# emreatilgan/P-Companion

Measured on AMD Instinct MI355X. Metric: triplets/sec (Product2Vec pretrain step: gather+fwd+bwd+Adam) + P-Companion joint step under `joint`, higher is better.
Workload: dtype f32

## Files before the change

### include/pcompanion_hip.h

```cpp
#ifndef PCOMPANION_HIP_H
#define PCOMPANION_HIP_H

#include <stddef.h>
#include <stdint.h>

#ifdef __cplusplus
extern "C" {
#endif

#define PC_OK 0
#define PC_EINVAL (-1)
#define PC_ESHAPE (-2)
#define PC_EWORKSPACE (-3)
#define PC_EBATCHNORM (-4)
#define PC_ECOMM (-5)

#define PC_D 128
#define PC_H 256
#define PC_HEADS 4
#define PC_L 64
#define PC_MAX_SEG 4
#define PC_BN_SYNC_DOUBLES (PC_MAX_SEG * 2 * 256 + PC_MAX_SEG)

#define PC_ABI_VERSION 8
int pc_abi_version(void);
enum { PC_OPT_SIDE_QUEUE = 1, PC_OPT_SORTED_TABLE_GRADIENTS = 2, PC_OPT_BN_FINALIZE_SIDE = 3, PC_OPT_FUSED_LOSS = 4,
       PC_OPT_FUSED_OUT_CHAIN = 5, PC_OPT_BN_FINALIZE_RIDES = 6, PC_OPT_DW0_STAGED_H = 7 };
int pc_set_option(int option, int value);
int pc_get_option(int option, int* value);
int pc_release_device_state(void);
enum {
    PC_FLAG_EXP_NO_MFMA = 1, PC_FLAG_EXP_NO_SPLIT = 2, PC_FLAG_EXP_NO_LDSREAD = 4, PC_FLAG_EXP_NO_DMA = 8,
    PC_FLAG_EXP_NO_SLAB = 16, PC_FLAG_EXP_STAGGER = 32, PC_FLAG_EXP_DMA_L2 = 64, PC_FLAG_NT_TIMING = 128,
    PC_FLAG_JOINT_TIMING = 256, PC_FLAG_CHAIN_TIMING = 512, PC_FLAG_EXP_NO_BARRIER = 1024, PC_FLAG_EXP_NO_VMWAIT = 2048
};
unsigned pc_build_flags(void);

typedef struct {
    float p;
    uint64_t seed, offset;
} pc_dropout;

typedef struct {
    float *w0, *b0, *gamma, *beta, *w3, *b3, *w5, *b5;
    float *in_proj_w, *in_proj_b, *out_proj_w, *out_proj_b;
    float *running_mean, *running_var;
    int64_t *num_batches_tracked;
    pc_dropout dropout;
    int dim;
} pc_p2v_tensors;

typedef struct {
    int nseg;
    int start[PC_MAX_SEG + 1];
    int count[PC_MAX_SEG];
    int weighted_row;
    float weight;
    const float *row_weight;
    int row_weight_start, row_weight_rows;
} pc_segments;

typedef struct {
    float *h0;
    float *a2;
    float *bn_mean;
    float *bn_invstd;
    float *bn_scale;
    float *bn_shift;
    float *a1;
} pc_ffn_saved;

size_t pc_p2v_ffn_workspace_bytes(int rows);
int pc_p2v_ffn_forward_train(const pc_p2v_tensors *p, const float *table, const int32_t *idx,
                             int rows, const pc_segments *seg, int update_running,
                             float *y, const pc_ffn_saved *saved, void *ws, size_t ws_bytes,
                             void *stream);

int pc_p2v_ffn_forward_eval(const pc_p2v_tensors *p, const float *table, const int32_t *idx,
                            int rows, float *y, void *ws, size_t ws_bytes, void *stream);

// ... 596 lines not shown
```

### p_companion_amd/_lib.py

```python
import ctypes
import os

_HERE = os.path.dirname(os.path.abspath(__file__))
LIB_PATH = os.path.join(_HERE, "libpcompanion_hip.so")
if os.environ.get("PC_DEV_LIB"):
    import sys as _sys
    LIB_PATH = os.path.abspath(os.environ["PC_DEV_LIB"])
    print(f"[p_companion_amd] PC_DEV_LIB: loading {LIB_PATH} instead of the in-tree library (developer A/B run)", file=_sys.stderr, flush=True)

c_f32p = ctypes.c_void_p
c_i32p = ctypes.c_void_p
PC_MAX_SEG = 4
D, H, HEADS, L = 128, 256, 4, 64

_ERR = {-1: "PC_EINVAL (null pointer / bad size)", -2: "PC_ESHAPE (unsupported dimension/alignment)",
        -3: "PC_EWORKSPACE (workspace too small)",
        -4: "PC_EBATCHNORM (a BatchNorm call group of one row in training mode)",
        -5: "PC_ECOMM (RCCL could not be loaded, or a communicator call failed)"}


class HipKernelError(RuntimeError):
    pass


# ... 1 lines not shown
    _fields_ = [("p", ctypes.c_float), ("seed", ctypes.c_uint64), ("offset", ctypes.c_uint64)]


class P2VTensors(ctypes.Structure):
    _fields_ = [(n, ctypes.c_void_p) for n in (
        "w0", "b0", "gamma", "beta", "w3", "b3", "w5", "b5", "in_proj_w", "in_proj_b", "out_proj_w",
        "out_proj_b", "running_mean", "running_var", "num_batches_tracked")] + [("dropout", Dropout), ("dim", ctypes.c_int)]


class Segments(ctypes.Structure):
    _fields_ = [("nseg", ctypes.c_int), ("start", ctypes.c_int * (PC_MAX_SEG + 1)),
                ("count", ctypes.c_int * PC_MAX_SEG), ("weighted_row", ctypes.c_int), ("weight", ctypes.c_float),
                ("row_weight", ctypes.c_void_p), ("row_weight_start", ctypes.c_int), ("row_weight_rows", ctypes.c_int)]


class FfnSaved(ctypes.Structure):
    _fields_ = [(n, ctypes.c_void_p) for n in ("h0", "a2", "bn_mean", "bn_invstd", "bn_scale", "bn_shift", "a1")]


class AttnSaved(ctypes.Structure):
    _fields_ = [(n, ctypes.c_void_p) for n in ("q", "qt", "probs", "c", "sp", "ctx")]


class JointTensors(ctypes.Structure):
    _fields_ = [(n, ctypes.c_void_p) for n in (
        "product_table", "enc_w", "enc_b", "dec_w", "dec_b", "typ_w", "typ_b", "itm_w", "itm_b",
        "query_types", "comp_types")] + [("dropout", Dropout)]


class JointSaved(ctypes.Structure):
    _fields_ = [(n, ctypes.c_void_p) for n in ("h", "c", "pi", "tp")]


_vp, _i, _sz, _f, _d, _u64, _i64 = (ctypes.c_void_p, ctypes.c_int, ctypes.c_size_t, ctypes.c_float,
                                    ctypes.c_double, ctypes.c_uint64, ctypes.c_int64)
_P = ctypes.POINTER

class AdamFused(ctypes.Structure):
    _fields_ = [("param", ctypes.c_void_p), ("grad", ctypes.c_void_p), ("exp_avg", ctypes.c_void_p), ("exp_avg_sq", ctypes.c_void_p),
                ("n", ctypes.c_size_t), ("step_count", ctypes.c_void_p), ("t", ctypes.c_int64),
                ("lr", ctypes.c_double), ("beta1", ctypes.c_double), ("beta2", ctypes.c_double), ("eps", ctypes.c_double)]


class RowWhere(ctypes.Structure):
    _fields_ = [(n, ctypes.c_void_p) for n in ("value", "lo", "hi", "flags", "need", "deny")]


PC_OPT_SIDE_QUEUE = 1
PC_OPT_FUSED_OUT_CHAIN = 5
PC_OPT_FUSED_LOSS = 4
PC_OPT_BN_FINALIZE_SIDE = 3
PC_OPT_BN_FINALIZE_RIDES = 6
PC_OPT_DW0_STAGED_H = 7
PC_OPT_SORTED_TABLE_GRADIENTS = 2

SIGNATURES = {
    "pc_abi_version": (_i, []),
    "pc_build_flags": (ctypes.c_uint, []),
    "pc_set_option": (_i, [_i, _i]),
    "pc_get_option": (_i, [_i, ctypes.POINTER(ctypes.c_int)]),
    "pc_release_device_state": (_i, []),
    "pc_p2v_ffn_workspace_bytes": (_sz, [_i]),
    "pc_p2v_ffn_forward_train": (_i, [_P(P2VTensors), _vp, _vp, _i, _P(Segments), _i, _vp, _P(FfnSaved), _vp, _sz, _vp]),
    "pc_p2v_ffn_forward_eval": (_i, [_P(P2VTensors), _vp, _vp, _i, _vp, _vp, _sz, _vp]),
    "pc_p2v_ffn_backward": (_i, [_P(P2VTensors), _P(P2VTensors), _vp, _vp, _i, _P(Segments), _vp, _P(FfnSaved),
                                 _vp, _i, _vp, _sz, _vp]),
    "pc_p2v_attention_workspace_bytes": (_sz, [_i, _i]),
    "pc_p2v_attention_workspace_bytes_dim": (_sz, [_i, _i, _i]),
    "pc_p2v_attention_forward": (_i, [_P(P2VTensors), _vp, _vp, _i, _i, _vp, _P(AttnSaved), _vp, _sz, _vp]),
    "pc_p2v_attention_backward": (_i, [_P(P2VTensors), _P(P2VTensors), _vp, _vp, _i, _i, _vp, _P(AttnSaved), _vp,
                                       _vp, _i, _vp, _sz, _vp]),
    "pc_p2v_attention_forward_masked": (_i, [_P(P2VTensors), _vp, _vp, _vp, _i, _i, _vp, _P(AttnSaved), _vp, _sz, _vp]),
    "pc_p2v_attention_backward_masked": (_i, [_P(P2VTensors), _P(P2VTensors), _vp, _vp, _vp, _i, _i, _vp, _P(AttnSaved), _vp,
                                              _vp, _i, _vp, _sz, _vp]),
    "pc_p2v_train_step_compact_masked": (_i, [_P(P2VTensors), _P(P2VTensors), _vp, _vp, _vp, _vp, _vp, _i, _vp, _i, _i, _i, _f,
                                              _vp, _vp, _vp, _vp, _vp, _vp, _sz, _vp]),
    "pc_p2v_train_step_unique_masked": (_i, [_P(P2VTensors), _P(P2VTensors), _vp, _vp, _vp, _vp, _vp, _vp, _vp, _i, _i, _vp, _vp,
                                             _vp, _i, _i, _i, _f, _vp, _vp, _vp, _vp, _vp, _vp, _sz, _P(AdamFused), _vp]),
    "pc_p2v_export_workspace_bytes": (_sz, [_i, _i]),
    "pc_p2v_export_embeddings": (_i, [_P(P2VTensors), _vp, _i64, _vp, _vp, _vp, _vp, _i, _vp, _sz, _vp]),
    "pc_p2v_triplet_loss": (_i, [_vp, _vp, _vp, _i, _i, _f, _vp, _vp, _vp, _vp, _vp, _vp, _vp]),
    "pc_p2v_triplet_loss_dim": (_i, [_vp, _vp, _vp, _i, _i, _i, _f, _vp, _vp, _vp, _vp, _vp, _vp, _vp]),
    "pc_adam_step": (_i, [_vp, _vp, _vp, _vp, _sz, _vp, _vp, _d, _d, _d, _d, _vp]),
    "pc_adam_step_at": (_i, [_vp, _vp, _vp, _vp, _sz, _vp, _i64, _d, _d, _d, _d, _vp]),
    "pc_p2v_train_step_workspace_bytes": (_sz, [_i, _i, _i]),
    "pc_p2v_train_step_workspace_bytes_dim": (_sz, [_i, _i, _i, _i]),
    "pc_p2v_train_step": (_i, [_P(P2VTensors), _P(P2VTensors), _vp, _vp, _vp, _vp, _vp, _i, _i, _i, _f, _vp, _vp,
                               _vp, _vp, _vp, _vp, _sz, _vp]),
    "pc_p2v_train_step_compact": (_i, [_P(P2VTensors), _P(P2VTensors), _vp, _vp, _vp, _vp, _vp, _i, _vp, _i, _i, _i, _f,
                                       _vp, _vp, _vp, _vp, _vp, _vp, _sz, _vp]),
    "pc_p2v_train_step_unique_adam": (_i, [_P(P2VTensors), _P(P2VTensors), _vp, _vp, _vp, _vp, _vp, _vp, _i, _vp, _vp, _vp, _i, _i,
                                           _i, _f, _vp, _vp, _vp, _vp, _vp, _vp, _sz, _P(AdamFused), _vp]),
    "pc_p2v_concat_step_rows": (_i, [_vp, _vp, _vp, _vp, _vp, _i, _i, _i, _vp, _i, _vp]),
    "pc_p2v_train_step_unique_rows": (_i, [_P(P2VTensors), _P(P2VTensors), _vp, _vp, _vp, _vp, _i, _vp, _vp, _vp, _i, _i,
                                           _i, _f, _vp, _vp, _vp, _vp, _vp, _vp, _sz, _P(AdamFused), _vp]),
    "pc_p2v_train_step_unique": (_i, [_P(P2VTensors), _P(P2VTensors), _vp, _vp, _vp, _vp, _vp, _vp, _i, _vp, _vp, _vp, _i, _i,
                                      _i, _f, _vp, _vp, _vp, _vp, _vp, _i, _vp, _vp, _vp, _vp, _sz, _vp]),
    "pc_build_similarity_batch_unique_scratch_bytes": (_sz, [_i, _i]),
    "pc_build_similarity_batch_unique": (_i, [_vp, _i, _vp, _vp, _vp, _vp, _vp, _i, _i, _i, _u64, _u64, _i, _vp, _vp, _vp,
                                              _vp, _vp, _vp, _vp, _vp, _vp, _vp, _sz, _vp]),
    "pc_p2v_train_step_compact_sync": (_i, [_P(P2VTensors), _P(P2VTensors), _vp, _vp, _vp, _vp, _vp, _i, _vp, _i, _i, _i,
                                            _f, _vp, _vp, _vp, _vp, _i, _vp, _vp, _vp, _vp, _sz, _vp]),
    "pc_build_similarity_batch_compact": (_i, [_vp, _i, _vp, _vp, _vp, _vp, _vp, _i, _i, _i, _u64, _u64, _vp, _vp, _vp,
                                               _vp, _vp, _vp, _vp]),
    "pc_profile_create": (_i, [_i, _P(ctypes.c_void_p)]),
    "pc_profile_destroy": (_i, [_vp]),
# ... 210 lines not shown
```

### p_companion_amd/csrc/common.h

```cpp
#pragma once
#include <hip/hip_runtime.h>
#include <stdint.h>
#include "../../include/pcompanion_hip.h"

typedef float f32x16 __attribute__((ext_vector_type(16)));
typedef float f32x4 __attribute__((ext_vector_type(4)));

#define PC_WAVE 64

#define PC_HIP_TRY(expr)                          \
    do {                                          \
        hipError_t _e = (expr);                   \
        if (_e != hipSuccess) return (int)_e;     \
    } while (0)

#define PC_TRY(expr)                 \
    do {                             \
        int _r = (expr);             \
        if (_r != 0) return _r;      \
    } while (0)

extern thread_local int pc_tls_launch_err;
#define PC_LAUNCH(...)                                                           \
    do {                                                                         \
// ... 466 lines not shown
};
struct TnReduceGroup {
    const float* slabs[PC_TN_RGROUP]; float* dW[PC_TN_RGROUP]; float* db[PC_TN_RGROUP];
    int nsplit[PC_TN_RGROUP], n_w[PC_TN_RGROUP], n_b[PC_TN_RGROUP], accumulate[PC_TN_RGROUP], block0[PC_TN_RGROUP + 1], n;
    AdamRider ad;
};
#define PC_FORK_EVENTS 3
struct PcFork { hipStream_t side; hipEvent_t fork[PC_FORK_EVENTS]; hipEvent_t join[PC_FORK_EVENTS]; int pending; };
PcFork* pc_fork_get(hipStream_t main_st);
int pc_fork_begin(PcFork* f, int i, hipStream_t main_st);
int pc_fork_mark(PcFork* f, int i);
int pc_fork_wait(PcFork* f, int i, hipStream_t main_st);
int pc_fork_join(PcFork* f, int i, hipStream_t main_st);
struct TnDefer { TnReduceGroup r; int rblocks; PcFork* fork; int bn_finalized; const pc_adam_fused* adam; };
static_assert(sizeof(TnGroup) <= 4096, "kernel argument segment");
int launch_gemm_tn_group(const TnArgs* args, int n, const TnReduceJob* extra, int n_extra, hipStream_t st,
                         TnDefer* defer = nullptr);
int launch_tn_reduce_deferred(TnDefer* d, hipStream_t st);
static inline void tn_defer_init(TnDefer* d) { d->r = TnReduceGroup{}; d->rblocks = 0; d->fork = nullptr; d->bn_finalized = 0; d->adam = nullptr; }
int scatter_add_slab_blocks(int table_rows, int rows, int width);
int launch_scatter_add_slabs(const int32_t* idx, int rows, int width, int table_rows, const float* src, float* slabs,
                             hipStream_t st);

struct WsCarver {
    char* base; size_t total;
    explicit WsCarver(void* b) : base(static_cast<char*>(b)), total(0) {}
    void* bytes(size_t n) {
        void* p = base ? base + total : nullptr;
        total += (n + 255) & ~(size_t)255;
        return p;
    }
    float* floats(size_t n) { return static_cast<float*>(bytes(n * sizeof(float))); }
};

static inline void joint_fields(const pc_joint_tensors* t, float* (&out)[10]) {
    float* const f[10] = {t->itm_w, t->itm_b, t->typ_w, t->typ_b, t->dec_w, t->dec_b, t->enc_w, t->enc_b, t->comp_types, t->query_types};
    for (int i = 0; i < 10; i++) out[i] = f[i];
}
static inline bool joint_tensors_ok(const pc_joint_tensors* t, bool need_table) {
    if (!t || (need_table && !t->product_table)) return false;
    float* f[10];
    joint_fields(t, f);
    for (float* x : f)
        if (!x) return false;
    return true;
}

int pc_opt_sorted_tables();
int pc_opt_bn_finalize_side();
int pc_opt_bn_finalize_rides();
int pc_opt_fused_loss();
int pc_opt_fused_out_chain();
int pc_opt_dw0_staged_h();
int triplet_loss_launch(const float* a, const float* p, const float* n, int batch, int k_neg, int dim, float margin,
                        float* loss, float* d_pos, float* d_neg, float* da, float* dp, float* dn, void* stream, int with_mean);
int launch_dropout(const float* x, size_t n, const pc_dropout& d, unsigned stream_id, float* y, hipStream_t st);
int launch_transpose(const float* in, int rows, int cols, float* out, hipStream_t st);
struct FfnCall {
    const pc_p2v_tensors *p = nullptr, *g = nullptr;
    const float* table = nullptr;
    const int32_t* idx = nullptr;
    int rows = 0;
    const pc_segments* seg = nullptr;
    const pc_ffn_saved* sv = nullptr;
    void* ws = nullptr; size_t ws_bytes = 0; void* stream = nullptr;
    double* local_sums = nullptr; const double* global_sums = nullptr;
    int update_running = 0; float* y = nullptr;
    const TransposeBatch* ride = nullptr;
    const float* dy = nullptr; float* dx = nullptr;
    int with_dx = 0, transposed = 0;
    int accumulate = 0;
    TnDefer* defer = nullptr;
};
int ffn_forward_part1(const FfnCall& c);
int ffn_forward_part2(const FfnCall& c);
int ffn_backward_part1(const FfnCall& c);
int ffn_backward_part2(const FfnCall& c);
int ffn_transposes(const pc_p2v_tensors* p, void* ws, int rows, int with_dx, TransposeBatch* tb);
int attention_transposes(const pc_p2v_tensors* p, void* ws, int B, int N, int key_rows, TransposeBatch* tb, float* zero_bk);
struct AttnCall {
    const pc_p2v_tensors* p = nullptr;
    const float *query = nullptr, *keys = nullptr;
    int B = 0, N = 0, key_rows = 0;
    const int32_t* slot_row = nullptr;
    const pc_attn_saved* sv = nullptr;
    void* ws = nullptr; size_t ws_bytes = 0; void* stream = nullptr;
    bool transposed = false;
    bool masked = false;
    const uint8_t* key_pad = nullptr;
    float* out = nullptr;
    const pc_p2v_tensors* g = nullptr;
    int pad_row = -1;
    const float* dout = nullptr;
    float *dquery = nullptr, *dkeys = nullptr;
    int accumulate = 0;
    const int32_t *ref_off = nullptr, *ref_slot = nullptr;
    TnDefer* defer = nullptr;
    const HingeMeanJob* rider = nullptr;
    const LossPro* loss = nullptr;
    const NtArgs* fwd_out_chain = nullptr;
    NtArgs* defer_out_chain = nullptr;
};
int attention_forward_impl(const AttnCall& c);
int attention_backward_impl(const AttnCall& c);

static inline NtArgs nt_plain(const float* A, int lda, const float* W, int ldw, const float* bias, float* C, int ldc, int M,
// ... 9 lines not shown
```

### p_companion_amd/csrc/gemm_tn.hip

```cpp
#include <atomic>
#include <mutex>
#include <type_traits>
#include "common.h"
#include "bn_finalize.h"
#include "lds_dma.h"

#define TM 128
#define TK 32

__device__ __forceinline__ float4 bn_bwd_z4(float4 z, const float4& h, float zm, const float4& mu, const float4& is,
                                            const float4& sc, const float4& c1, const float4& c2) {
    z.x = sc.x * (z.x - zm * (c1.x + (h.x - mu.x) * is.x * c2.x));
    z.y = sc.y * (z.y - zm * (c1.y + (h.y - mu.y) * is.y * c2.y));
    z.z = sc.z * (z.z - zm * (c1.z + (h.z - mu.z) * is.z * c2.z));
    z.w = sc.w * (z.w - zm * (c1.w + (h.w - mu.w) * is.w * c2.w));
    return z;
}

__device__ __forceinline__ void tn_small_body(const TnArgs& a, int tiles_i, int nsplit, int rows_per_split, int bid) {
    __shared__ __attribute__((aligned(16))) float smem[2][2][TK * TM];

    const int tid = threadIdx.x, lane = tid & 63, w = tid >> 6, wo = w >> 1, wi = w & 1;
    const int split = bid % nsplit;
    const int tile = bid / nsplit;
// ... 89 lines not shown
            const float x0 = As[k * TM], x1 = As[k * TM + 32];
            if (vz0 && vx0) acc[0][0] = mfma32(z0, x0, acc[0][0]);
            if (vz0 && vx1) acc[0][1] = mfma32(z0, x1, acc[0][1]);
            if (vz1 && vx0) acc[1][0] = mfma32(z1, x0, acc[1][0]);
            if (vz1 && vx1) acc[1][1] = mfma32(z1, x1, acc[1][1]);
        }
        if (c + 1 < nchunk) lstore(cur ^ 1);
        __syncthreads();
    }

    float* slab = a.slabs + (size_t)split * ((size_t)a.No * a.Ni + a.No);
#pragma unroll
    for (int mt = 0; mt < 2; mt++)
#pragma unroll
        for (int nt = 0; nt < 2; nt++) {
            const int i = i0 + wi * 64 + nt * 32 + (lane & 31);
#pragma unroll
            for (int reg = 0; reg < 16; reg++) {
                const int o = o0 + wo * 64 + mt * 32 + (reg & 3) + 8 * (reg >> 2) + 4 * (lane >> 5);
                if (o < a.No && i < a.Ni) slab[(size_t)o * a.Ni + i] = acc[mt][nt][reg];
            }
        }
    if (a.db && i0 == 0) {
        float* red = &smem[0][0][0];
        *reinterpret_cast<float4*>(&red[lrow * TM + lcol]) = dbacc;
        __syncthreads();
        if (tid < TM && o0 + tid < a.No) {
            float s = 0.f;
#pragma unroll
            for (int g = 0; g < 8; g++) s += red[g * TM + tid];
            slab[(size_t)a.No * a.Ni + o0 + tid] = s;
        }
    }
}

__global__ __launch_bounds__(256, 2) void gemm_tn_kernel(TnArgs a, int tiles_i, int nsplit, int rows_per_split) {
    tn_small_body(a, tiles_i, nsplit, rows_per_split, blockIdx.x);
}

__global__ __launch_bounds__(256, 2) void gemm_tn_group_kernel(TnGroup g) {
    const int b = blockIdx.x;
    int j = 0;
#pragma unroll
    for (int i = 1; i < PC_TN_GROUP; i++) j += (i < g.n && b >= g.block0[i]) ? 1 : 0;
    tn_small_body(g.a[j], g.tiles_i[j], g.nsplit[j], g.rps[j], b - g.block0[j]);
}

__device__ __attribute__((aligned(64))) float pc_tn_zero_chunk[16];

struct TnNoRider {};
typedef float tn_v4f __attribute__((ext_vector_type(4)));
__device__ __forceinline__ void tn_tie_h(tn_v4f (&h)[4]) { asm volatile("" : "+v"(h[0]), "+v"(h[1]), "+v"(h[2]), "+v"(h[3])::"memory"); }
__device__ __forceinline__ void tn_tie_h(tn_v4f (&h)[2]) { asm volatile("" : "+v"(h[0]), "+v"(h[1])::"memory"); }
#ifdef PC_EXP_DW0_REGH_16X3
#define PC_TN_REGH_ALL 1
#else
#define PC_TN_REGH_ALL 0
#endif
template <int WO, int WI, int TO, int TI, int TKC, int NST, bool APRO, bool ZPRO, bool RIDER = false>
__global__ __launch_bounds__(64 * WO * WI, WO * WI / 4) void gemm_tn8_kernel(TnArgs a, int nsplit, int rows_per_split, int halves,
                                                                             size_t slab_half_off,
                                                                             std::conditional_t<RIDER, TnRider, TnNoRider> rider) {
    constexpr bool REGH = ZPRO && (TKC == 32 || (PC_TN_REGH_ALL && WO == 4));
    static_assert(!REGH || (!APRO && !RIDER), "register H is a form of the ZPRO loader");
    constexpr int NWV = WO * WI, THREADS = 64 * NWV;
    constexpr int NO = WO * TO * 32, NI = WI * TI * 32;
    constexpr int ZRS = NO == 256 ? 260 : NO, ARS = NI == 256 ? 260 : NI;
    constexpr bool ZSW = NO == 128, ASW = NI == 128;
    static_assert((NO == 128 || NO == 256) && (NI == 128 || NI == 256), "image widths");
    constexpr int ZF = TKC * ZRS, AF = TKC * ARS;
    constexpr int ZIMG = (ZPRO && !REGH) ? 2 : 1;
    constexpr int STAGE = ZF * ZIMG + AF;
    constexpr int JZ = TKC * NO / 256 / NWV, JA = TKC * NI / 256 / NWV;
    static_assert((TKC * NO) % (256 * NWV) == 0 && (TKC * NI) % (256 * NWV) == 0, "images must split into whole wave instructions over the waves");
    constexpr int JALL = JZ * ZIMG + JA;
    __shared__ __attribute__((aligned(1024))) float smem[NST * STAGE];

    const int tid = threadIdx.x, lane = tid & 63;
    const int w = __builtin_amdgcn_readfirstlane(tid >> 6), wo = w % WO, wi = w / WO;
    const int half = halves == 2 ? ((int)blockIdx.x >> 3) & 1 : 0;
    const int split = halves == 2 ? (((int)blockIdx.x >> 4) << 3) + ((int)blockIdx.x & 7) : (int)blockIdx.x;
    if (halves == 2) {
        a.Z += half * (WO * TO * 32);
        a.slabs += half * slab_half_off;
        if (a.db) a.db += half * (WO * TO * 32);
    }
    const int r_begin = split * rows_per_split;
    const int r_end = min(a.R, r_begin + rows_per_split);
    const float* const zsrc0 = pc_tn_zero_chunk;
    const unsigned lds0 = (unsigned)(uintptr_t)(lptr_t)&smem[0];
    if constexpr (RIDER) {
        int rid = -1;
#pragma unroll
        for (int i = 0; i < PC_TN_RIDERS; i++) rid = (int)blockIdx.x == rider.block[i] ? i : rid;
        if (rid >= 0) {
            static_assert(sizeof(smem) >= sizeof(BnFinBwdScratch) && THREADS == FIN4_CG * FIN4_LANES, "a finalize workgroup");
            bn_finalize_bwd_body(rider.fin, rider.si, rid, (int)threadIdx.x, reinterpret_cast<BnFinBwdScratch*>(smem));
            return;
        }
    }

    int zr[JZ], zc[JZ], ar[JA], ac[JA];
    unsigned zd[JZ], ad[JA];
#pragma unroll
    for (int j = 0; j < JZ; j++) {
        const int g = w + NWV * j, f = g * 256 + lane * 4;
        zr[j] = f / NO; zc[j] = f % NO;
        if (ZSW && (zr[j] & 8)) zc[j] ^= 32;
        zd[j] = (NO == 256 ? g * ZRS : g * 256) * 4;
    }
#pragma unroll
    for (int j = 0; j < JA; j++) {
        const int g = w + NWV * j, f = g * 256 + lane * 4;
        ar[j] = f / NI; ac[j] = f % NI;
        if (ASW && (ar[j] & 8)) ac[j] ^= 32;
        ad[j] = (NI == 256 ? g * ARS : g * 256) * 4;
    }
    int gidx[JA];
    auto load_gather = [&](int r0) {
#pragma unroll
        for (int j = 0; j < JA; j++) {
            const int r = r0 + ar[j];
            gidx[j] = (a.gather && r < r_end) ? a.gather[r] : r;
        }
    };
    auto issue = [&](int st, int r0) {
        const unsigned base = lds0 + st * (STAGE * 4);
#pragma unroll
        for (int j = 0; j < JZ; j++) {
            const int r = r0 + zr[j];
            const bool v = r < r_end && zc[j] < a.No;
            dma16(v ? a.Z + (size_t)r * a.ldz + zc[j] : zsrc0, base + zd[j]);
            if (ZIMG == 2) dma16(v ? a.zaux + (size_t)r * a.ldzaux + zc[j] : zsrc0, base + ZF * 4 + zd[j]);
        }
#pragma unroll
        for (int j = 0; j < JA; j++) {
            const int r = r0 + ar[j];
            const bool v = r < r_end && ac[j] < a.Ni && gidx[j] >= 0;
            dma16(v ? a.A + (size_t)gidx[j] * a.lda + ac[j] : zsrc0, base + ZIMG * ZF * 4 + ad[j]);
        }
    };

    constexpr int ZT = NO / 4, AT = NI / 4;
    const int zrow = tid / ZT, zcol = (tid % ZT) * 4, arow = tid / AT, acol = (tid % AT) * 4;
    int zseg = -1;
    float4 zmu, zis, zsc, zc1, zc2;
    constexpr int HP = TKC / (THREADS / ZT);
    [[maybe_unused]] tn_v4f hreg[HP];
    [[maybe_unused]] float hmult[HP];
    [[maybe_unused]] auto load_h = [&](int r0) {
#pragma unroll
        for (int p = 0; p < HP; p++) {
            const int r = r0 + zrow + (THREADS / ZT) * p;
            const bool v = r < r_end && zcol < a.No;
            const float* src = v ? a.zaux + (size_t)r * a.ldzaux + zcol : zsrc0;
            asm volatile("global_load_dwordx4 %0, %1, off" : "=v"(hreg[p]) : "v"(src) : "memory");
            hmult[p] = *(v ? row_multiplicity_src(a.seg, r, zsrc0) : zsrc0);
        }
    };
    auto transform = [&](float* stage, int r0) {
        if (ZPRO && zcol < a.No) {
            float* Zs = stage;
            const float* Hs = stage + ZF;
#pragma unroll
            for (int p = 0; p < HP; p++) {
                const int rr = zrow + (THREADS / ZT) * p, r = r0 + rr;
                if (r < r_end) {
                    const int s = seg_of_row(a.seg, r);
                    if (s != zseg) {
                        const size_t o = (size_t)s * a.No + zcol;
                        zmu = *reinterpret_cast<const float4*>(a.z_mean + o);
                        zis = *reinterpret_cast<const float4*>(a.z_invstd + o);
                        zsc = *reinterpret_cast<const float4*>(a.z_scale + o);
                        zc1 = *reinterpret_cast<const float4*>(a.z_c1 + o);
                        zc2 = *reinterpret_cast<const float4*>(a.z_c2 + o);
                        zseg = s;
                    }
                    const int zp = rr * ZRS + ((ZSW && (rr & 8)) ? zcol ^ 32 : zcol);
                    const float4 z = *reinterpret_cast<const float4*>(&Zs[zp]);
                    float4 h;
                    if constexpr (REGH) h = make_float4(hreg[p].x, hreg[p].y, hreg[p].z, hreg[p].w);
                    else h = *reinterpret_cast<const float4*>(&Hs[zp]);
                    float zm;
                    if constexpr (REGH) zm = row_multiplicity_from(a.seg, r, hmult[p]);
                    else zm = row_multiplicity(a.seg, r);
                    *reinterpret_cast<float4*>(&Zs[zp]) = bn_bwd_z4(z, h, zm, zmu, zis, zsc, zc1, zc2);
                }
            }
        }
        if (APRO && acol < a.Ni) {
            float* As = stage + ZIMG * ZF;
            int aseg = -1;
            float4 asc, ash;
#pragma unroll
            for (int p = 0; p < TKC / (THREADS / AT); p++) {
                const int rr = arow + (THREADS / AT) * p, r = r0 + rr;
                if (r < r_end) {
                    const int s = seg_of_row(a.seg, r);
                    if (s != aseg) {
                        asc = *reinterpret_cast<const float4*>(a.pscale + (size_t)s * a.Ni + acol);
                        ash = *reinterpret_cast<const float4*>(a.pshift + (size_t)s * a.Ni + acol);
                        aseg = s;
                    }
                    const int ap = rr * ARS + ((ASW && (rr & 8)) ? acol ^ 32 : acol);
                    float4 x = *reinterpret_cast<const float4*>(&As[ap]);
                    x.x = fast_tanh(x.x * asc.x + ash.x);
                    x.y = fast_tanh(x.y * asc.y + ash.y);
                    x.z = fast_tanh(x.z * asc.z + ash.z);
                    x.w = fast_tanh(x.w * asc.w + ash.w);
                    *reinterpret_cast<float4*>(&As[ap]) = x;
                }
            }
        }
    };

    f32x16 acc[TO][TI];
    float zsum[TO];
#pragma unroll
    for (int i = 0; i < TO; i++) {
        zsum[i] = 0.f;
#pragma unroll
        for (int j = 0; j < TI; j++)
#pragma unroll
            for (int r = 0; r < 16; r++) acc[i][j][r] = 0.f;
    }

    const int nchunk = (r_end - r_begin + TKC - 1) / TKC;
#pragma unroll
    for (int i = 0; i < NST - 1; i++)
        if (i < nchunk) { load_gather(r_begin + i * TKC); issue(i, r_begin + i * TKC); }
    if (NST - 1 < nchunk) load_gather(r_begin + (NST - 1) * TKC);
    if constexpr (REGH) {
        if (nchunk > 0) {
            load_h(r_begin);
            asm volatile("s_waitcnt vmcnt(0)" ::: "memory");
            tn_tie_h(hreg);
        }
    }
    static_assert(TKC % 16 == 0, "chunks are whole k groups");
    const int fz = 8 * (lane >> 5) * ZRS, fa = 8 * (lane >> 5) * ARS;
    int zo[TO], xo[TI];
#pragma unroll
    for (int i = 0; i < TO; i++) zo[i] = (wo * (TO * 32) + 32 * i + (lane & 31)) ^ ((ZSW && lane >= 32) ? 32 : 0);
#pragma unroll
    for (int j = 0; j < TI; j++) xo[j] = (wi * (TI * 32) + 32 * j + (lane & 31)) ^ ((ASW && lane >= 32) ? 32 : 0);
    int cur = 0;
    for (int c = 0; c < nchunk; c++) {
#ifndef PC_EXP_NO_VMWAIT
        if (c + NST - 1 <= nchunk) { asm volatile("s_waitcnt vmcnt(%0)" ::"n"((NST - 2) * JALL) : "memory"); }
        else { asm volatile("s_waitcnt vmcnt(0)" ::: "memory"); }
        if constexpr (REGH) {
            tn_tie_h(hreg);
#pragma unroll
            for (int j = 0; j < JA; j++) asm volatile("" : "+v"(gidx[j]));
        }
#endif
#ifndef PC_EXP_NO_BARRIER
        __syncthreads();
#endif
        if constexpr (REGH) {
            transform(smem + cur * STAGE, r_begin + c * TKC);
            if (c + 1 < nchunk) load_h(r_begin + (c + 1) * TKC);
        }
#ifndef PC_EXP_NO_DMA
        if (c + NST - 1 < nchunk) {
            issue(cur == 0 ? NST - 1 : cur - 1, r_begin + (c + NST - 1) * TKC);
            if (c + NST < nchunk) load_gather(r_begin + (c + NST) * TKC);
        }
#endif
        float* stage = smem + cur * STAGE;
        if constexpr (REGH) lds_sync();
        else if (APRO || ZPRO) { transform(stage, r_begin + c * TKC); lds_sync(); }
        const float* Zs = stage + fz;
        const float* As = stage + ZIMG * ZF + fa;
#pragma unroll
        for (int g = 0; g < TKC / 16; g++) {
#if defined(PC_EXP_NO_LDSREAD)
#define PC_TNV(PTR, OFF) __int_as_float(a.R + t)
#else
#define PC_TNV(PTR, OFF) (PTR)[OFF]
#endif
            Split3 sx[TI];
#pragma unroll
            for (int j = 0; j < TI; j++) {
                float v[8];
#pragma unroll
                for (int t = 0; t < 8; t++) v[t] = PC_TNV(As, (16 * g + t) * ARS + xo[j]);
                sx[j] = PC_SPLIT(make_float4(v[0], v[1], v[2], v[3]), make_float4(v[4], v[5], v[6], v[7]));
            }
#pragma unroll
            for (int i = 0; i < TO; i++) {
                float v[8];
#pragma unroll
                for (int t = 0; t < 8; t++) v[t] = PC_TNV(Zs, (16 * g + t) * ZRS + zo[i]);
                zsum[i] += ((v[0] + v[1]) + (v[2] + v[3])) + ((v[4] + v[5]) + (v[6] + v[7]));
                const Split3 sz = PC_SPLIT(make_float4(v[0], v[1], v[2], v[3]), make_float4(v[4], v[5], v[6], v[7]));
#define PC_TERM(PZ, PX) _Pragma("unroll") for (int j = 0; j < TI; j++) acc[i][j] = PC_MFMA(sz.PZ, sx[j].PX, acc[i][j]);
                PC_PRIO_MFMA(PC_PRIO_TN_COND, 1);
                PC_TERM(p2, p0) PC_TERM(p0, p2) PC_TERM(p1, p1) PC_TERM(p1, p0) PC_TERM(p0, p1) PC_TERM(p0, p0)
                PC_PRIO_MFMA(PC_PRIO_TN_COND, 0);
#undef PC_TERM
            }
        }
        cur = cur + 1 == NST ? 0 : cur + 1;
    }

    float* slab = a.slabs + (size_t)split * ((size_t)a.No * a.Ni + a.No);
#pragma unroll
    for (int i = 0; i < TO; i++)
#pragma unroll
        for (int j = 0; j < TI; j++) {
            const int ci = wi * (TI * 32) + j * 32 + (lane & 31);
#pragma unroll
            for (int reg = 0; reg < 16; reg++) {
                const int o = wo * (TO * 32) + i * 32 + (reg & 3) + 8 * (reg >> 2) + 4 * (lane >> 5);
#ifdef PC_EXP_NO_SLAB
                if (o < a.No && ci < a.Ni && acc[i][j][reg] == 12345.678f) slab[(size_t)o * a.Ni + ci] = acc[i][j][reg];
#else
                if (o < a.No && ci < a.Ni) slab[(size_t)o * a.Ni + ci] = acc[i][j][reg];
#endif
            }
        }
    if (a.db && wi == 0) {
#pragma unroll
        for (int i = 0; i < TO; i++) {
            const float s = zsum[i] + __shfl_xor(zsum[i], 32, 64);
            const int o = wo * (TO * 32) + i * 32 + (lane & 31);
            if (lane < 32 && o < a.No) slab[(size_t)a.No * a.Ni + o] = s;
        }
    }
}

__device__ __forceinline__ void adam_rider4(const AdamRider& ad, size_t off, const float4 gv, float step_size, float bc2s) {
    float4 pv = *reinterpret_cast<float4*>(ad.p + off);
    float4 mv = *reinterpret_cast<float4*>(ad.m + off);
    float4 vv = *reinterpret_cast<float4*>(ad.v + off);
    if (pc_adam_dead(gv, mv, vv)) return;
#define ADAM1(c) pc_adam_update(pv.c, mv.c, vv.c, gv.c, step_size, bc2s, ad.omb1, ad.beta2f, ad.omb2, ad.eps);
    ADAM1(x) ADAM1(y) ADAM1(z) ADAM1(w)
#undef ADAM1
    *reinterpret_cast<float4*>(ad.p + off) = pv;
    *reinterpret_cast<float4*>(ad.m + off) = mv;
    *reinterpret_cast<float4*>(ad.v + off) = vv;
}

__device__ __forceinline__ void tn_reduce_body(const float* slabs, int nsplit, int n_w, int n_b, float* dW, float* db,
                                               int accumulate, int bid, const AdamRider* ad = nullptr, float step_size = 0.f,
                                               float bc2s = 0.f) {
    const int total4 = (n_w + (db ? n_b : 0)) / 4;
    const int t = bid * blockDim.x + threadIdx.x;
    const int j4 = t >> 3, g = t & 7;
    if (j4 >= total4) return;
    const size_t stride = (size_t)n_w + n_b;
    const float* src = slabs + (size_t)j4 * 4;
    float4 s = make_float4(0.f, 0.f, 0.f, 0.f);
// ... 65 lines not shown
    } else {
        const int tiles = ((No + TM - 1) / TM) * ((Ni + TM - 1) / TM);
        s = (512 + tiles - 1) / tiles;
    }
    const int max_s = (R + 63) / 64;
    if (s > max_s) s = max_s;
    if (s < 1) s = 1;
    int rps = (R + s - 1) / s;
    rps = (rps + TK - 1) / TK * TK;
    s = (R + rps - 1) / rps;
    *nsplit = s;
    *rows_per_split = rps;
}

size_t gemm_tn_workspace_floats(int R, int No, int Ni) {
    const int tiles = ((No + TM - 1) / TM) * ((Ni + TM - 1) / TM);
    int cap = (512 + tiles - 1) / tiles;
    if (No <= 256 && Ni <= 256 && (No > 128 || Ni > 128) && No % 64 == 0 && Ni % 64 == 0 && cap < 256) cap = 256;
    int s = (R + 63) / 64;
    if (s > cap) s = cap;
    if (s < 1) s = 1;
    return (size_t)s * ((size_t)No * Ni + No);
}

static int tn_defer_push(TnDefer* d, const float* slabs, size_t slab_floats, int nsplit, int n_w, int n_b, float* dW,
                         float* db, int accumulate) {
    if (d->r.n >= PC_TN_RGROUP) return PC_EINVAL;
    const size_t used = (size_t)nsplit * ((size_t)n_w + n_b);
    if (used > slab_floats) return PC_EWORKSPACE;
    for (int k = 0; k < d->r.n; k++) {
        const float* lo = d->r.slabs[k];
        const float* hi = lo + (size_t)d->r.nsplit[k] * ((size_t)d->r.n_w[k] + d->r.n_b[k]);
        if (slabs < hi && lo < slabs + used) return PC_EINVAL;
    }
    const int k = d->r.n++;
    d->r.slabs[k] = slabs; d->r.nsplit[k] = nsplit; d->r.n_w[k] = n_w; d->r.n_b[k] = n_b; d->r.dW[k] = dW; d->r.db[k] = db;
    d->r.accumulate[k] = accumulate; d->r.block0[k] = d->rblocks;
    d->rblocks += ((n_w + (db ? n_b : 0)) / 4 * 8 + 255) / 256;
    return PC_OK;
}

int launch_gemm_tn(const TnArgs& a, hipStream_t st, TnDefer* defer) {
    if ((!a.Z && !a.z_onehot) || !a.A || !a.dW || !a.slabs || a.R <= 0 || a.No <= 0 || a.Ni <= 0) return PC_EINVAL;
    if (a.No % 4 || a.Ni % 4 || (a.Z && a.ldz % 4) || a.lda % 4 || a.lddw != a.Ni) return PC_ESHAPE;
    if (a.z_onehot && (a.zaux || tn_full_tile(a.R, a.No, a.Ni))) return PC_ESHAPE;
    if (((uintptr_t)a.dW & 15) || (a.db && ((uintptr_t)a.db & 15)) || ((uintptr_t)a.slabs & 15)) return PC_ESHAPE;
    int nsplit, rps;
    tn_plan(a.R, a.No, a.Ni, &nsplit, &rps);
    if ((size_t)nsplit * ((size_t)a.No * a.Ni + a.No) > a.slab_floats) return PC_EWORKSPACE;
    const int tiles_o = (a.No + TM - 1) / TM, tiles_i = (a.Ni + TM - 1) / TM;
    const bool apro = a.prologue == NT_PRO_BNTANH, zpro = a.zaux != nullptr;
    const int pb = pc_prof_begin(PC_KIND_GEMM_TN, 2.0 * a.R * (double)a.No * a.Ni, st);
    if (tn_full_tile(a.R, a.No, a.Ni) && !(apro && zpro)) {
#if PC_TN_REGH_ALL
#define TN8_REGH gemm_tn8_kernel<4, 2, 2, 2, 16, 3, false, true>
#else
#define TN8_REGH gemm_tn8_kernel<4, 2, 2, 2, 32, 2, false, true>
#endif
#define TN8(WO, WI, TO, TI, TKC, NST)                                                                         \
    do {                                                                                                      \
        if (apro) PC_LAUNCH((gemm_tn8_kernel<WO, WI, TO, TI, TKC, NST, true, false>), dim3(nsplit), dim3(64 * WO * WI), 0, st, a, nsplit, rps, 1, (size_t)0, TnNoRider{});    \
        else if (zpro && a.Ni > 128) PC_LAUNCH((gemm_tn8_kernel<2, 4, 4, 2, 16, 3, false, true>), dim3(nsplit), dim3(512), 0, st, a, nsplit, rps, 1, (size_t)0, TnNoRider{});  \
        else if (zpro && !pc_opt_dw0_staged_h()) PC_LAUNCH((TN8_REGH), dim3(nsplit), dim3(512), 0, st, a, nsplit, rps, 1, (size_t)0, TnNoRider{});  \
        else if (zpro) PC_LAUNCH((gemm_tn8_kernel<4, 2, 2, 2, 16, 3, false, true>), dim3(nsplit), dim3(512), 0, st, a, nsplit, rps, 1, (size_t)0, TnNoRider{});  \
        else PC_LAUNCH((gemm_tn8_kernel<WO, WI, TO, TI, TKC, NST, false, false>), dim3(nsplit), dim3(64 * WO * WI), 0, st, a, nsplit, rps, 1, (size_t)0, TnNoRider{});        \
    } while (0)
        if (a.No > 128 && a.Ni > 128) TN8(2, 4, 4, 2, 16, 3);
        else if (a.No > 128) TN8(4, 2, 2, 2, 32, 2);
        else TN8(2, 4, 2, 2, 32, 2);
#undef TN8
#undef TN8_REGH
    } else {
        PC_LAUNCH(gemm_tn_kernel, dim3(tiles_o * tiles_i * nsplit), dim3(256), 0, st, a, tiles_i, nsplit, rps);
    }
    pc_prof_end(pb, st);
    PC_TRY(pc_launch_status());
    const int n_w = a.No * a.Ni, n_b = a.No;
    const int threads = (n_w + (a.db ? n_b : 0)) / 4 * 8;
    if (defer) return tn_defer_push(defer, a.slabs, a.slab_floats, nsplit, n_w, n_b, a.dW, a.db, a.accumulate);
    PC_LAUNCH(tn_reduce_kernel, dim3((threads + 255) / 256), dim3(256), 0, st, a.slabs, nsplit, n_w, n_b,
                       a.dW, a.db, a.accumulate);
    return pc_launch_status();
}

int launch_gemm_tn_halves(const TnArgs& a, float* slabs0, float* slabs1, size_t slab_floats, hipStream_t st, TnDefer* defer,
                          const TnRider* rider) {
    if (!a.Z || !a.A || !a.dW || !slabs0 || !slabs1 || !defer || a.R <= 0) return PC_EINVAL;
    if (a.No != 256 || a.Ni != 256 || a.ldz % 4 || a.lda % 4 || a.lddw != a.Ni || a.prologue != NT_PRO_NONE || a.zaux || a.z_onehot || a.gather)
        return PC_ESHAPE;
    if (slabs1 < slabs0) return PC_EINVAL;
    const int nsplit = 128;
    int rps = (a.R + nsplit - 1) / nsplit;
    rps = (rps + 31) / 32 * 32;
    const int used = (a.R + rps - 1) / rps;
    const size_t per = (size_t)128 * a.Ni + 128;
    if ((size_t)nsplit * per > slab_floats) return PC_EWORKSPACE;
    TnArgs h = a;
    h.No = 128; h.slabs = slabs0; h.slab_floats = slab_floats;
    TnRider rd = {};
    int blocks = 2 * nsplit, nred = nsplit;
    if (rider && rider->n) {
        if (rider->n != PC_TN_RIDERS) return PC_EINVAL;
        rd = *rider;
        int k = 0;
        for (int b = 0; b < 2 * nsplit && k < rd.n; b++)
            if (((b >> 4) << 3) + (b & 7) >= used) rd.block[k++] = b;
        if (k == rd.n) nred = used;
        else {
            for (k = 0; k < rd.n; k++) rd.block[k] = blocks + k;
            blocks += rd.n;
        }
    }
    const int pb = pc_prof_begin(PC_KIND_GEMM_TN, 2.0 * a.R * (double)a.No * a.Ni, st);
    if (rd.n)
        PC_LAUNCH((gemm_tn8_kernel<2, 4, 2, 2, 32, 2, false, false, true>), dim3(blocks), dim3(512), 0, st, h, nsplit, rps, 2,
                  (size_t)(slabs1 - slabs0), rd);
    else
        PC_LAUNCH((gemm_tn8_kernel<2, 4, 2, 2, 32, 2, false, false>), dim3(blocks), dim3(512), 0, st, h, nsplit, rps, 2,
                  (size_t)(slabs1 - slabs0), TnNoRider{});
    pc_prof_end(pb, st);
    PC_TRY(pc_launch_status());
    PC_TRY(tn_defer_push(defer, slabs0, slab_floats, nred, 128 * a.Ni, 128, a.dW, a.db, a.accumulate));
    return tn_defer_push(defer, slabs1, slab_floats, nred, 128 * a.Ni, 128, a.dW + (size_t)128 * a.Ni, a.db ? a.db + 128 : nullptr,
                         a.accumulate);
}

namespace {
struct ForkSlot { int dev; hipStream_t main_st; int state; PcFork f; };
ForkSlot g_fork_slots[32];
std::mutex g_fork_mu;
std::atomic<int> g_opt_side_queue{1};
std::atomic<int> g_opt_sorted_tables{1};
std::atomic<int> g_opt_bn_finalize_side{0};
std::atomic<int> g_opt_bn_finalize_rides{1};
std::atomic<int> g_opt_fused_loss{1};
std::atomic<int> g_opt_fused_out_chain{1};
std::atomic<int> g_opt_dw0_staged_h{0};
std::atomic<int>* opt_slot(int option) {
    switch (option) {
        case PC_OPT_DW0_STAGED_H: return &g_opt_dw0_staged_h;
        case PC_OPT_SIDE_QUEUE: return &g_opt_side_queue;
        case PC_OPT_SORTED_TABLE_GRADIENTS: return &g_opt_sorted_tables;
        case PC_OPT_BN_FINALIZE_SIDE: return &g_opt_bn_finalize_side;
        case PC_OPT_FUSED_LOSS: return &g_opt_fused_loss;
        case PC_OPT_FUSED_OUT_CHAIN: return &g_opt_fused_out_chain;
        case PC_OPT_BN_FINALIZE_RIDES: return &g_opt_bn_finalize_rides;
        default: return nullptr;
    }
}
}
int pc_opt_sorted_tables() { return g_opt_sorted_tables.load(std::memory_order_relaxed); }
int pc_opt_bn_finalize_side() { return g_opt_bn_finalize_side.load(std::memory_order_relaxed); }
int pc_opt_bn_finalize_rides() { return g_opt_bn_finalize_rides.load(std::memory_order_relaxed); }
int pc_opt_fused_loss() { return g_opt_fused_loss.load(std::memory_order_relaxed); }
int pc_opt_fused_out_chain() { return g_opt_fused_out_chain.load(std::memory_order_relaxed); }
int pc_opt_dw0_staged_h() { return g_opt_dw0_staged_h.load(std::memory_order_relaxed); }

extern "C" int pc_set_option(int option, int value) {
    std::atomic<int>* o = opt_slot(option);
    if (!o || (value != 0 && value != 1)) return PC_EINVAL;
    o->store(value, std::memory_order_relaxed);
    return PC_OK;
}
extern "C" int pc_get_option(int option, int* value) {
    std::atomic<int>* o = opt_slot(option);
    if (!o || !value) return PC_EINVAL;
    *value = o->load(std::memory_order_relaxed);
    return PC_OK;
}
extern "C" int pc_release_device_state(void) {
    std::lock_guard<std::mutex> lock(g_fork_mu);
    int cur = 0, rc = PC_OK;
    const bool have_cur = hipGetDevice(&cur) == hipSuccess;
    for (ForkSlot& c : g_fork_slots) {
        if (c.state == 1) {
            if (hipSetDevice(c.dev) != hipSuccess) { rc = (int)hipErrorInvalidDevice; continue; }
            (void)hipStreamSynchronize(c.f.side);
            for (int i = 0; i < PC_FORK_EVENTS; i++) { (void)hipEventDestroy(c.f.fork[i]); (void)hipEventDestroy(c.f.join[i]); }
            (void)hipStreamDestroy(c.f.side);
        }
        c = ForkSlot{};
    }
    if (have_cur) (void)hipSetDevice(cur);
    return rc;
}

PcFork* pc_fork_get(hipStream_t main_st) {
    int dev = 0;
    if (!g_opt_side_queue.load(std::memory_order_relaxed) || hipGetDevice(&dev) != hipSuccess) return nullptr;
    hipStreamCaptureStatus cap = hipStreamCaptureStatusNone;
    if (hipStreamIsCapturing(main_st, &cap) != hipSuccess || cap != hipStreamCaptureStatusNone) return nullptr;
    std::lock_guard<std::mutex> lock(g_fork_mu);
    ForkSlot* s = nullptr;
    for (ForkSlot& c : g_fork_slots) {
        if (c.state != 0 && c.dev == dev && c.main_st == main_st) { s = &c; break; }
        if (c.state == 0 && !s) s = &c;
    }
    if (!s) return nullptr;
    if (s->state == 0) {
        s->dev = dev; s->main_st = main_st;
        PcFork& f = s->f;
        int prio = 0;
        bool ok = (hipStreamGetPriority(main_st, &prio) == hipSuccess
                       ? hipStreamCreateWithPriority(&f.side, hipStreamNonBlocking, prio)
                       : hipStreamCreateWithFlags(&f.side, hipStreamNonBlocking)) == hipSuccess;
        for (int i = 0; ok && i < PC_FORK_EVENTS; i++)
            ok = hipEventCreateWithFlags(&f.fork[i], hipEventDisableTiming) == hipSuccess &&
                 hipEventCreateWithFlags(&f.join[i], hipEventDisableTiming) == hipSuccess;
        f.pending = 0;
// ... 153 lines not shown
```

Measured before the change: 5.557 million.

## Make deep 16x3 register-H pipeline the default dW0 backward GEMM form

Adds a deeper register-H variant of the TN GEMM for the dW0 weight gradient. It uses 16-row chunks with three stages and issues the gather index, multiplicity and H loads one chunk ahead through inline asm, with explicit vmcnt waits. This form replaces the previous 32x2 register-H kernel as the default, and the old form stays reachable through a new option. The aim is to hide global-load latency for the BN-backward prologue behind the MFMA work. The cost is more registers and hand-tuned wait counts that only hold for Ni <= 128.

After: 5.576 million (median of 4 runs). No clear change (+0.3%).

```diff
diff --git a/include/pcompanion_hip.h b/include/pcompanion_hip.h
--- a/include/pcompanion_hip.h
+++ b/include/pcompanion_hip.h
@@ -25,7 +25,8 @@
 #define PC_ABI_VERSION 8
 int pc_abi_version(void);
 enum { PC_OPT_SIDE_QUEUE = 1, PC_OPT_SORTED_TABLE_GRADIENTS = 2, PC_OPT_BN_FINALIZE_SIDE = 3, PC_OPT_FUSED_LOSS = 4,
-       PC_OPT_FUSED_OUT_CHAIN = 5, PC_OPT_BN_FINALIZE_RIDES = 6, PC_OPT_DW0_STAGED_H = 7 };
+       PC_OPT_FUSED_OUT_CHAIN = 5, PC_OPT_BN_FINALIZE_RIDES = 6, PC_OPT_DW0_STAGED_H = 7,
+       PC_OPT_DW0_REGH_32X2 = 8 };
 int pc_set_option(int option, int value);
 int pc_get_option(int option, int* value);
 int pc_release_device_state(void);
diff --git a/p_companion_amd/_lib.py b/p_companion_amd/_lib.py
--- a/p_companion_amd/_lib.py
+++ b/p_companion_amd/_lib.py
@@ -77,6 +77,7 @@
 PC_OPT_BN_FINALIZE_SIDE = 3
 PC_OPT_BN_FINALIZE_RIDES = 6
 PC_OPT_DW0_STAGED_H = 7
+PC_OPT_DW0_REGH_32X2 = 8
 PC_OPT_SORTED_TABLE_GRADIENTS = 2
 
 SIGNATURES = {
diff --git a/p_companion_amd/csrc/common.h b/p_companion_amd/csrc/common.h
--- a/p_companion_amd/csrc/common.h
+++ b/p_companion_amd/csrc/common.h
@@ -542,6 +542,7 @@
 int pc_opt_fused_loss();
 int pc_opt_fused_out_chain();
 int pc_opt_dw0_staged_h();
+int pc_opt_dw0_regh_32x2();
 int triplet_loss_launch(const float* a, const float* p, const float* n, int batch, int k_neg, int dim, float margin,
                         float* loss, float* d_pos, float* d_neg, float* da, float* dp, float* dn, void* stream, int with_mean);
 int launch_dropout(const float* x, size_t n, const pc_dropout& d, unsigned stream_id, float* y, hipStream_t st);
diff --git a/p_companion_amd/csrc/gemm_tn.hip b/p_companion_amd/csrc/gemm_tn.hip
--- a/p_companion_amd/csrc/gemm_tn.hip
+++ b/p_companion_amd/csrc/gemm_tn.hip
@@ -165,17 +165,14 @@
 typedef float tn_v4f __attribute__((ext_vector_type(4)));
 __device__ __forceinline__ void tn_tie_h(tn_v4f (&h)[4]) { asm volatile("" : "+v"(h[0]), "+v"(h[1]), "+v"(h[2]), "+v"(h[3])::"memory"); }
 __device__ __forceinline__ void tn_tie_h(tn_v4f (&h)[2]) { asm volatile("" : "+v"(h[0]), "+v"(h[1])::"memory"); }
-#ifdef PC_EXP_DW0_REGH_16X3
-#define PC_TN_REGH_ALL 1
-#else
-#define PC_TN_REGH_ALL 0
-#endif
-template <int WO, int WI, int TO, int TI, int TKC, int NST, bool APRO, bool ZPRO, bool RIDER = false>
+__device__ __forceinline__ void tn_tie_deep(tn_v4f (&h)[2], float (&m)[2], int (&g)[1]) {
+    asm volatile("" : "+v"(h[0]), "+v"(h[1]), "+v"(m[0]), "+v"(m[1]), "+v"(g[0])::"memory");
+}
+template <int WO, int WI, int TO, int TI, int TKC, int NST, bool APRO, bool ZPRO, bool REGH = false, bool RIDER = false>
 __global__ __launch_bounds__(64 * WO * WI, WO * WI / 4) void gemm_tn8_kernel(TnArgs a, int nsplit, int rows_per_split, int halves,
                                                                              size_t slab_half_off,
                                                                              std::conditional_t<RIDER, TnRider, TnNoRider> rider) {
-    constexpr bool REGH = ZPRO && (TKC == 32 || (PC_TN_REGH_ALL && WO == 4));
-    static_assert(!REGH || (!APRO && !RIDER), "register H is a form of the ZPRO loader");
+    static_assert(!REGH || (ZPRO && !APRO && !RIDER), "register H is a form of the ZPRO loader");
     constexpr int NWV = WO * WI, THREADS = 64 * NWV;
     constexpr int NO = WO * TO * 32, NI = WI * TI * 32;
     constexpr int ZRS = NO == 256 ? 260 : NO, ARS = NI == 256 ? 260 : NI;
@@ -229,12 +226,27 @@
         if (ASW && (ar[j] & 8)) ac[j] ^= 32;
         ad[j] = (NI == 256 ? g * ARS : g * 256) * 4;
     }
+    constexpr bool DEEP = REGH && NST > 2;
+    static_assert(!DEEP || (NST == 3 && JA == 1), "the deep form's wait count and tie statement are written for 16 x 3 at Ni <= 128");
     int gidx[JA];
+    [[maybe_unused]] int gnext[JA] = {};
     auto load_gather = [&](int r0) {
 #pragma unroll
         for (int j = 0; j < JA; j++) {
             const int r = r0 + ar[j];
-            gidx[j] = (a.gather && r < r_end) ? a.gather[r] : r;
+            if constexpr (DEEP) {
+                const int32_t* src = (a.gather && r < r_end) ? a.gather + r : reinterpret_cast<const int32_t*>(zsrc0);
+                asm volatile("global_load_dword %0, %1, off" : "=v"(gnext[j]) : "v"(src) : "memory");
+            } else {
+                gidx[j] = (a.gather && r < r_end) ? a.gather[r] : r;
+            }
+        }
+    };
+    [[maybe_unused]] auto take_gather = [&](int r0) {
+#pragma unroll
+        for (int j = 0; j < JA; j++) {
+            const int r = r0 + ar[j];
+            gidx[j] = (a.gather && r < r_end) ? gnext[j] : r;
         }
     };
     auto issue = [&](int st, int r0) {
@@ -268,8 +280,15 @@
             const bool v = r < r_end && zcol < a.No;
             const float* src = v ? a.zaux + (size_t)r * a.ldzaux + zcol : zsrc0;
             asm volatile("global_load_dwordx4 %0, %1, off" : "=v"(hreg[p]) : "v"(src) : "memory");
-            hmult[p] = *(v ? row_multiplicity_src(a.seg, r, zsrc0) : zsrc0);
-        }
+            const float* msrc = v ? row_multiplicity_src(a.seg, r, zsrc0) : zsrc0;
+            if constexpr (DEEP) asm volatile("global_load_dword %0, %1, off" : "=v"(hmult[p]) : "v"(msrc) : "memory");
+            else hmult[p] = *msrc;
+        }
+    };
+    [[maybe_unused]] auto load_coef = [&](const float* src) {
+        tn_v4f v;
+        asm volatile("global_load_dwordx4 %0, %1, off" : "=v"(v) : "v"(src) : "memory");
+        return v;
     };
     auto transform = [&](float* stage, int r0) {
         if (ZPRO && zcol < a.No) {
@@ -282,11 +301,23 @@
                     const int s = seg_of_row(a.seg, r);
                     if (s != zseg) {
                         const size_t o = (size_t)s * a.No + zcol;
-                        zmu = *reinterpret_cast<const float4*>(a.z_mean + o);
-                        zis = *reinterpret_cast<const float4*>(a.z_invstd + o);
-                        zsc = *reinterpret_cast<const float4*>(a.z_scale + o);
-                        zc1 = *reinterpret_cast<const float4*>(a.z_c1 + o);
-                        zc2 = *reinterpret_cast<const float4*>(a.z_c2 + o);
+                        if constexpr (DEEP) {
+                            tn_v4f c[5] = {load_coef(a.z_mean + o), load_coef(a.z_invstd + o), load_coef(a.z_scale + o),
+                                           load_coef(a.z_c1 + o), load_coef(a.z_c2 + o)};
+                            asm volatile("s_waitcnt vmcnt(0)" ::: "memory");
+                            asm volatile("" : "+v"(c[0]), "+v"(c[1]), "+v"(c[2]), "+v"(c[3]), "+v"(c[4])::"memory");
+                            zmu = make_float4(c[0].x, c[0].y, c[0].z, c[0].w);
+                            zis = make_float4(c[1].x, c[1].y, c[1].z, c[1].w);
+                            zsc = make_float4(c[2].x, c[2].y, c[2].z, c[2].w);
+                            zc1 = make_float4(c[3].x, c[3].y, c[3].z, c[3].w);
+                            zc2 = make_float4(c[4].x, c[4].y, c[4].z, c[4].w);
+                        } else {
+                            zmu = *reinterpret_cast<const float4*>(a.z_mean + o);
+                            zis = *reinterpret_cast<const float4*>(a.z_invstd + o);
+                            zsc = *reinterpret_cast<const float4*>(a.z_scale + o);
+                            zc1 = *reinterpret_cast<const float4*>(a.z_c1 + o);
+                            zc2 = *reinterpret_cast<const float4*>(a.z_c2 + o);
+                        }
                         zseg = s;
                     }
                     const int zp = rr * ZRS + ((ZSW && (rr & 8)) ? zcol ^ 32 : zcol);
@@ -341,9 +372,24 @@
     const int nchunk = (r_end - r_begin + TKC - 1) / TKC;
 #pragma unroll
     for (int i = 0; i < NST - 1; i++)
-        if (i < nchunk) { load_gather(r_begin + i * TKC); issue(i, r_begin + i * TKC); }
-    if (NST - 1 < nchunk) load_gather(r_begin + (NST - 1) * TKC);
-    if constexpr (REGH) {
+        if (i < nchunk) {
+            load_gather(r_begin + i * TKC);
+            if constexpr (DEEP) {
+                asm volatile("s_waitcnt vmcnt(0)" ::: "memory");
+                asm volatile("" : "+v"(gnext[0])::"memory");
+                take_gather(r_begin + i * TKC);
+            }
+            issue(i, r_begin + i * TKC);
+        }
+    if constexpr (DEEP) {
+        load_gather(r_begin + (NST - 1) * TKC);
+        load_h(r_begin);
+        asm volatile("s_waitcnt vmcnt(0)" ::: "memory");
+        tn_tie_deep(hreg, hmult, gnext);
+    } else {
+        if (NST - 1 < nchunk) load_gather(r_begin + (NST - 1) * TKC);
+    }
+    if constexpr (REGH && !DEEP) {
         if (nchunk > 0) {
             load_h(r_begin);
             asm volatile("s_waitcnt vmcnt(0)" ::: "memory");
@@ -359,10 +405,16 @@
     for (int j = 0; j < TI; j++) xo[j] = (wi * (TI * 32) + 32 * j + (lane & 31)) ^ ((ASW && lane >= 32) ? 32 : 0);
     int cur = 0;
     for (int c = 0; c < nchunk; c++) {
+        if constexpr (DEEP) {
+            take_gather(r_begin + (c + NST - 1) * TKC);
+            asm volatile("" : "+v"(gidx[0]));
+        }
 #ifndef PC_EXP_NO_VMWAIT
-        if (c + NST - 1 <= nchunk) { asm volatile("s_waitcnt vmcnt(%0)" ::"n"((NST - 2) * JALL) : "memory"); }
-        else { asm volatile("s_waitcnt vmcnt(0)" ::: "memory"); }
-        if constexpr (REGH) {
+        if constexpr (!DEEP) {
+            if (c + NST - 1 <= nchunk) { asm volatile("s_waitcnt vmcnt(%0)" ::"n"((NST - 2) * JALL) : "memory"); }
+            else { asm volatile("s_waitcnt vmcnt(0)" ::: "memory"); }
+        }
+        if constexpr (REGH && !DEEP) {
             tn_tie_h(hreg);
 #pragma unroll
             for (int j = 0; j < JA; j++) asm volatile("" : "+v"(gidx[j]));
@@ -373,12 +425,17 @@
 #endif
         if constexpr (REGH) {
             transform(smem + cur * STAGE, r_begin + c * TKC);
-            if (c + 1 < nchunk) load_h(r_begin + (c + 1) * TKC);
+            if constexpr (DEEP) {
+                load_h(r_begin + (c + 1) * TKC);
+                load_gather(r_begin + (c + NST) * TKC);
+            } else {
+                if (c + 1 < nchunk) load_h(r_begin + (c + 1) * TKC);
+            }
         }
 #ifndef PC_EXP_NO_DMA
-        if (c + NST - 1 < nchunk) {
+        if (DEEP || c + NST - 1 < nchunk) {
             issue(cur == 0 ? NST - 1 : cur - 1, r_begin + (c + NST - 1) * TKC);
-            if (c + NST < nchunk) load_gather(r_begin + (c + NST) * TKC);
+            if constexpr (!DEEP) { if (c + NST < nchunk) load_gather(r_begin + (c + NST) * TKC); }
         }
 #endif
         float* stage = smem + cur * STAGE;
@@ -414,6 +471,10 @@
                 PC_PRIO_MFMA(PC_PRIO_TN_COND, 0);
 #undef PC_TERM
             }
+        }
+        if constexpr (DEEP) {
+            asm volatile("s_waitcnt vmcnt(%0)" ::"n"(JALL) : "memory");
+            tn_tie_deep(hreg, hmult, gnext);
         }
         cur = cur + 1 == NST ? 0 : cur + 1;
     }
@@ -585,24 +646,20 @@
     const bool apro = a.prologue == NT_PRO_BNTANH, zpro = a.zaux != nullptr;
     const int pb = pc_prof_begin(PC_KIND_GEMM_TN, 2.0 * a.R * (double)a.No * a.Ni, st);
     if (tn_full_tile(a.R, a.No, a.Ni) && !(apro && zpro)) {
-#if PC_TN_REGH_ALL
-#define TN8_REGH gemm_tn8_kernel<4, 2, 2, 2, 16, 3, false, true>
-#else
-#define TN8_REGH gemm_tn8_kernel<4, 2, 2, 2, 32, 2, false, true>
-#endif
 #define TN8(WO, WI, TO, TI, TKC, NST)                                                                         \
     do {                                                                                                      \
+        const int dw0_form = pc_opt_dw0_staged_h() ? 1 : pc_opt_dw0_regh_32x2() ? 2 : 0;                      \
         if (apro) PC_LAUNCH((gemm_tn8_kernel<WO, WI, TO, TI, TKC, NST, true, false>), dim3(nsplit), dim3(64 * WO * WI), 0, st, a, nsplit, rps, 1, (size_t)0, TnNoRider{});    \
         else if (zpro && a.Ni > 128) PC_LAUNCH((gemm_tn8_kernel<2, 4, 4, 2, 16, 3, false, true>), dim3(nsplit), dim3(512), 0, st, a, nsplit, rps, 1, (size_t)0, TnNoRider{});  \
-        else if (zpro && !pc_opt_dw0_staged_h()) PC_LAUNCH((TN8_REGH), dim3(nsplit), dim3(512), 0, st, a, nsplit, rps, 1, (size_t)0, TnNoRider{});  \
-        else if (zpro) PC_LAUNCH((gemm_tn8_kernel<4, 2, 2, 2, 16, 3, false, true>), dim3(nsplit), dim3(512), 0, st, a, nsplit, rps, 1, (size_t)0, TnNoRider{});  \
+        else if (zpro && dw0_form == 0) PC_LAUNCH((gemm_tn8_kernel<4, 2, 2, 2, 16, 3, false, true, true>), dim3(nsplit), dim3(512), 0, st, a, nsplit, rps, 1, (size_t)0, TnNoRider{});  \
+        else if (zpro && dw0_form == 1) PC_LAUNCH((gemm_tn8_kernel<4, 2, 2, 2, 16, 3, false, true>), dim3(nsplit), dim3(512), 0, st, a, nsplit, rps, 1, (size_t)0, TnNoRider{});  \
+        else if (zpro) PC_LAUNCH((gemm_tn8_kernel<4, 2, 2, 2, 32, 2, false, true, true>), dim3(nsplit), dim3(512), 0, st, a, nsplit, rps, 1, (size_t)0, TnNoRider{});  \
         else PC_LAUNCH((gemm_tn8_kernel<WO, WI, TO, TI, TKC, NST, false, false>), dim3(nsplit), dim3(64 * WO * WI), 0, st, a, nsplit, rps, 1, (size_t)0, TnNoRider{});        \
     } while (0)
         if (a.No > 128 && a.Ni > 128) TN8(2, 4, 4, 2, 16, 3);
         else if (a.No > 128) TN8(4, 2, 2, 2, 32, 2);
         else TN8(2, 4, 2, 2, 32, 2);
 #undef TN8
-#undef TN8_REGH
     } else {
         PC_LAUNCH(gemm_tn_kernel, dim3(tiles_o * tiles_i * nsplit), dim3(256), 0, st, a, tiles_i, nsplit, rps);
     }
@@ -646,7 +703,7 @@
     }
     const int pb = pc_prof_begin(PC_KIND_GEMM_TN, 2.0 * a.R * (double)a.No * a.Ni, st);
     if (rd.n)
-        PC_LAUNCH((gemm_tn8_kernel<2, 4, 2, 2, 32, 2, false, false, true>), dim3(blocks), dim3(512), 0, st, h, nsplit, rps, 2,
+        PC_LAUNCH((gemm_tn8_kernel<2, 4, 2, 2, 32, 2, false, false, false, true>), dim3(blocks), dim3(512), 0, st, h, nsplit, rps, 2,
                   (size_t)(slabs1 - slabs0), rd);
     else
         PC_LAUNCH((gemm_tn8_kernel<2, 4, 2, 2, 32, 2, false, false>), dim3(blocks), dim3(512), 0, st, h, nsplit, rps, 2,
@@ -669,9 +726,11 @@
 std::atomic<int> g_opt_fused_loss{1};
 std::atomic<int> g_opt_fused_out_chain{1};
 std::atomic<int> g_opt_dw0_staged_h{0};
+std::atomic<int> g_opt_dw0_regh_32x2{0};
 std::atomic<int>* opt_slot(int option) {
     switch (option) {
         case PC_OPT_DW0_STAGED_H: return &g_opt_dw0_staged_h;
+        case PC_OPT_DW0_REGH_32X2: return &g_opt_dw0_regh_32x2;
         case PC_OPT_SIDE_QUEUE: return &g_opt_side_queue;
         case PC_OPT_SORTED_TABLE_GRADIENTS: return &g_opt_sorted_tables;
         case PC_OPT_BN_FINALIZE_SIDE: return &g_opt_bn_finalize_side;
@@ -688,6 +747,7 @@
 int pc_opt_fused_loss() { return g_opt_fused_loss.load(std::memory_order_relaxed); }
 int pc_opt_fused_out_chain() { return g_opt_fused_out_chain.load(std::memory_order_relaxed); }
 int pc_opt_dw0_staged_h() { return g_opt_dw0_staged_h.load(std::memory_order_relaxed); }
+int pc_opt_dw0_regh_32x2() { return g_opt_dw0_regh_32x2.load(std::memory_order_relaxed); }
 
 extern "C" int pc_set_option(int option, int value) {
     std::atomic<int>* o = opt_slot(option);
```
